# LouisBearing/BirdSoundClassif

Hardware: AMD Instinct MI355X
Metric: clips/sec (3 s @ 22.05 kHz) detect fwd (higher is better)
Workload: dtype f32; 1 GPU; BASELINE.json configs[1]: 1xMI355X inference, batch=64 synthetic 3 s clips (PCM16 @22.05 kHz resident in HBM) through the HIP STFT front end + detector forward + device post-processing, detections returned to the host; batch_per_gpu=64, distinct_clips=64, lanes=2

## Files before the change

### birdsoundclassif_amd/_lib.py

```python
import ctypes as C
import os
import subprocess

_HERE = os.path.dirname(os.path.abspath(__file__))
LIB_PATH = os.environ.get('NBM_LIB') or os.path.join(_HERE, 'libnbm_hip.so')
CSRC = os.path.join(_HERE, 'csrc')

_lib = None


class GemmDesc(C.Structure):
    _fields_ = [('x', C.c_void_p), ('w', C.c_void_p), ('y', C.c_void_p),
                ('scale', C.c_void_p), ('shift', C.c_void_p), ('residual', C.c_void_p),
                ('x_gs', C.c_int64), ('w_gs', C.c_int64), ('y_gs', C.c_int64), ('res_gs', C.c_int64),
                ('groups', C.c_int),
                ('B', C.c_int), ('H', C.c_int), ('W', C.c_int), ('Cin', C.c_int),
                ('N', C.c_int),
                ('kh', C.c_int), ('kw', C.c_int), ('stride', C.c_int), ('pad', C.c_int),
                ('Ho', C.c_int), ('Wo', C.c_int),
                ('x_ld', C.c_int), ('w_ld', C.c_int), ('y_ld', C.c_int), ('res_ld', C.c_int),
                ('alpha', C.c_float), ('act', C.c_int), ('shift_per_row', C.c_int),
                ('up', C.c_void_p), ('up_H', C.c_int), ('up_W', C.c_int),
                ('rows', C.c_void_p), ('rows_blocks', C.c_void_p),
                ('rows_mode', C.c_int), ('rows_count', C.c_int), ('rows_TH', C.c_int), ('rows_TW', C.c_int),
# ... 83 lines not shown
    'nbm_silu': [_P, _P, _L, _P],
    'nbm_layernorm': [_P, _L, _I, _P, _P, _F, _P, _P],
    'nbm_mha_small': [_P, _P, _P, _I, _I, _I, _P, _I, _I, _I, _I, _I, _L, _L, _P, _F, _P],
    'nbm_mha_segments': [_P, _P, _P, _I, _I, _I, _P, _I, _I, _I, _I, _I, _I, _P, _P, _I, _F, _P],
    'nbm_pair_softmax': [_P, _L, _I, _I, _P, _I, _P],
    'nbm_rpn_decode': [_P, _P, _P, _I, _I, _I, _I, _I, _I, _P, _P, _P, _P],
    'nbm_nan_images': [_P, _I, _L, _P, _P],
    'nbm_rpn_select': [_P, _P, _P, _I, _I, _I, _I, _I, _P, _P, _P, _P, _P],
    'nbm_nms_batched': [_P, _P, _P, _I, _I, _F, _I, _P, _P, _P, _P, _P, _P, _P],
    'nbm_rpn_select_big_workspace': [_I, _I, C.POINTER(C.c_int64)],
    'nbm_rpn_select_big': [_P, _P, _P, _I, _I, _I, _I, _I, _P, _L, _P, _P, _P, _P, _P],
    'nbm_nms_big_workspace': [_I, _I, C.POINTER(C.c_int64)],
    'nbm_nms_big': [_P, _P, _P, _I, _I, _F, _I, _P, _L, _P, _P, _P, _P, _P],
    'nbm_roi_pool': [C.POINTER(RoiDesc), _P],
    'nbm_roi_pool_hw': [C.POINTER(RoiHwDesc), _P],
    'nbm_rcnn_post': [_P, _P, _I, _I, _P, _P, _I, _I, _I, _F, _F, _I, _P, _P, _P],
    'nbm_merge_collect': [_P, _P, _I, _I, _I, _I, _I, _L, _P, _P, _P, _P, _P, _P],
    'nbm_merge_nms_workspace': [_I, C.POINTER(C.c_int64)],
    'nbm_merge_nms': [_P, _P, _I, _F, _P, _L, _P, _P, _P],
    'nbm_merge_gather': [_P, _P, _P, _P, _P, _I, _P, _P, _P],
    'nbm_conv_dgrad': [C.POINTER(BwdDesc), _P],
    'nbm_conv_wgrad': [C.POINTER(BwdDesc), _P],
    'nbm_gemm_plan': [_I, _P, C.POINTER(GemmPlan)],
    'nbm_relu_bwd': [_P, _P, _P, _L, _P],
    'nbm_silu_bwd': [_P, _P, _P, _L, _P],
    'nbm_axpby': [_P, _P, _P, _F, _F, _L, _L, _P],
    'nbm_colsum': [_P, _L, _I, _I, _P, _P],
    'nbm_leaky_relu_bwd': [_P, _P, _P, _F, _L, _P],
    'nbm_layernorm_bwd': [_P, _P, _P, _L, _I, _F, _P, _P, _P, _P],
    'nbm_mha_small_bwd': [_P, _P, _P, _P, _I, _I, _I, _I, _P, _P, _P, _I, _I, _I, _P, _I, _I, _I, _I, _L, _L, _P, _F, _P],
    'nbm_zero_roi_windows': [_P, _I, _I, _I, _P, _P, _I, _I, _I, _P],
    'nbm_zero_pattern': [_P, _I, _I, _I, _I, _I, _P],
    'nbm_zero_tiles': [_P, _I, _I, _I, _I, _P, _I, _P, _P],
    'nbm_tiles_gather': [_P, _I, _I, _I, _I, _P, _I, _P, _P, _P],
    'nbm_tiles_scatter_add': [_P, _I, _I, _I, _I, _P, _I, _P, _P, _P],
    'nbm_proposal_iou': [_P, _P, _P, _I, _I, _I, _P, _P, _P],
    'nbm_anchor_targets': [_P, _I, _P, _P, _I, _I, _F, _F, _P, _P, _P, _P],
    'nbm_maxpool3x3s2_bwd': [_P, _P, _P, _I, _I, _I, _I, _I, _I, _P, _P, _P],
    'nbm_upsample_bilinear_bwd': [_P, _I, _I, _I, _I, _P, _I, _I, _I, _P],
    'nbm_tiles_upsample_bilinear_bwd_add': [_P, _I, _I, _I, _I, _P, _I, _P, _P, _I, _I, _P],
    'nbm_png_unfilter_gray8': [_P, _L, _I, _I, _I, _P, _L, _P, _P],
    'nbm_image_half_std_u8': [_P, _L, _I, _L, _P, _P],
    'nbm_randn_fill': [_U64, _L, _P, _P],
    'nbm_augment_batch': [_P, _P, _P, _I, _I, _I, _P, _P, _P, _P, _P, _P, _P],
    'nbm_u8_to_unit': [_P, _L, _P, _P],
    'nbm_wino_input': [_P, _I, _I, _I, _I, _P, _I, _P],
# ... 48 lines not shown
def load():
    global _lib
    if _lib is not None:
        return _lib
    import torch
    if not os.path.isfile(LIB_PATH):
        raise RuntimeError(f'{LIB_PATH} is missing: build it with `python -c "import __graft_entry__ as g; g.build()"` '
                           '(the NBM hot path has no CPU / eager fallback)')
    lib = C.CDLL(LIB_PATH)
    lib.nbm_version.restype = C.c_char_p
    lib.nbm_version.argtypes = []
    for name, argtypes in SIGNATURES.items():
        fn = getattr(lib, name)
        fn.argtypes = argtypes
        fn.restype = C.c_int
    _lib = lib
    return lib


class NbmHipError(RuntimeError):
    pass


_CODES = {-1: 'NBM_EINVAL (bad argument / shape)', -2: 'NBM_EALIGN (pointer or pitch not 16-byte aligned)',
          -3: 'NBM_EUNSUPPORTED'}


def check(rc, name):
    if rc != 0:
        raise NbmHipError(f'{name} failed: {_CODES.get(rc, f"hipError_t {rc}")}')
```

### birdsoundclassif_amd/csrc/igemm.hip

```cpp
#include <stdlib.h>
#include "nbm_common.h"
#include "igemm_device.h"
#include <type_traits>

namespace {

constexpr int BK = 32;
constexpr int PITCH = 36;

enum { A_FAST = 0, A_GENERIC = 1 };

using nbm_igemm::IgemmParams;

template <int BM, int BN, int WM, int WN, int AMODE, int EPI, int STAGES = 2, bool ROWS = false>
__global__ __launch_bounds__(256, BM > 128 ? 1 : STAGES == 1 ? 3 : 2) void igemm_kernel(const IgemmParams p) {
  constexpr int MT = WM / 32, NT = WN / 32;
  constexpr int WAVES_N = BN / WN;
  constexpr int AR = BM / 32, BR = BN / 32;
  static_assert((BM / WM) * (BN / WN) == 4, "4 waves per workgroup");
  static_assert(EPI == EPI_STD, "EPI is reserved: the instantiation names carry it");

  __shared__ __attribute__((aligned(16))) float lds[STAGES * (BM + BN) * PITCH];
  if constexpr (STAGES == 2) nbm_stagger_priority();
  float* As = lds;
// ... 351 lines not shown
      }
    }
    if (p.bits_out) {
      static_assert(NT >= 2 && NT % 2 == 0, "two lanes per tile row");
      constexpr int WPL = NT / 2;
      __builtin_amdgcn_fence(__ATOMIC_ACQ_REL, "wavefront");
      const int r = lane >> 1, j0 = (lane & 1) * WPL;
      const int m = m0 + r;
      if (m < p.M) {
        unsigned* dst = p.bits_out + (long long)m * p.n_words + (n_off >> 5) + j0;
        const unsigned* src = Bw[wave] + r * NT + j0;
        if constexpr (WPL == 4) *reinterpret_cast<uint4*>(dst) = *reinterpret_cast<const uint4*>(src);
        else if constexpr (WPL == 2) *reinterpret_cast<uint2*>(dst) = *reinterpret_cast<const uint2*>(src);
        else {
#pragma unroll
          for (int q = 0; q < WPL; ++q) dst[q] = src[q];
        }
      }
      __builtin_amdgcn_fence(__ATOMIC_ACQ_REL, "wavefront");
    }
  }
}

}

using namespace nbm_igemm;

extern "C" int nbm_gemm_conv(const nbm_gemm_desc* d, void* stream) {
  if (!d) return NBM_EINVAL;
  const GemmPlan pl = plan_fwd(*d, read_gemm_switches(0));
  if (pl.rc) return pl.rc;
  if (pl.halves) {
    nbm_gemm_desc a = *d, b = *d;
    const int n0 = d->N - 64;
    a.N = n0;
    b.N = 64;
    b.w = d->w + (long long)n0 * d->w_ld;
    b.y = d->y + n0;
    if (d->scale) b.scale = d->scale + n0;
    if (d->shift) b.shift = d->shift + n0;
    if (d->residual) b.residual = d->residual + n0;
    if (d->mask) b.mask = d->mask + n0;
    const int rc = nbm_gemm_conv(&a, stream);
    return rc ? rc : nbm_gemm_conv(&b, stream);
  }
  const dim3 grid(pl.grid[0], pl.grid[1], pl.grid[2]), block(pl.block);
// ... 30 lines not shown
  }
  if (d->rows) {
    p.rows = d->rows; p.rows_blocks = d->rows_blocks; p.rows_mode = d->rows_mode; p.rows_TH = d->rows_TH; p.rows_TW = d->rows_TW;
    p.fd_rows_thw = nbm_fastdiv_make((unsigned)(d->rows_TH * d->rows_TW)); p.fd_rows_tw = nbm_fastdiv_make((unsigned)d->rows_TW);
    p.M = d->rows_count;
  }
  switch (pl.kernel) {
    case K_FWD_ROWS: hipLaunchKernelGGL((igemm_kernel<128, 128, 64, 64, A_FAST, EPI_STD, 1, true>), grid, block, 0, st, p); break;
    case K_FWD_SPLIT_R0: case K_FWD_SPLIT_R2: case K_FWD_SPLIT_R4: return split_launch(p, pl, st);
    case K_FWD_H16: return h16_launch(p, pl, st);
    case K_FWD_128_S1: hipLaunchKernelGGL((igemm_kernel<128, 128, 64, 64, A_FAST, EPI_STD, 1>), grid, block, 0, st, p); break;
    case K_FWD_128_FAST: hipLaunchKernelGGL((igemm_kernel<128, 128, 64, 64, A_FAST, EPI_STD>), grid, block, 0, st, p); break;
    case K_FWD_128_GENERIC: hipLaunchKernelGGL((igemm_kernel<128, 128, 64, 64, A_GENERIC, EPI_STD>), grid, block, 0, st, p); break;
    case K_FWD_64_S1: hipLaunchKernelGGL((igemm_kernel<128, 64, 64, 32, A_FAST, EPI_STD, 1>), grid, block, 0, st, p); break;
    case K_FWD_64_FAST: hipLaunchKernelGGL((igemm_kernel<128, 64, 64, 32, A_FAST, EPI_STD>), grid, block, 0, st, p); break;
    case K_FWD_64_GENERIC: hipLaunchKernelGGL((igemm_kernel<128, 64, 64, 32, A_GENERIC, EPI_STD>), grid, block, 0, st, p); break;
    case K_FWD_32_FAST: hipLaunchKernelGGL((igemm_kernel<128, 32, 32, 32, A_FAST, EPI_STD>), grid, block, 0, st, p); break;
    case K_FWD_32_GENERIC: hipLaunchKernelGGL((igemm_kernel<128, 32, 32, 32, A_GENERIC, EPI_STD>), grid, block, 0, st, p); break;
    default: return NBM_EINVAL;
  }
  return nbm_launch_status();
}

extern "C" int nbm_gemm_plan(int kind, const void* desc, nbm_gemm_plan_t* out) {
  if (!desc || !out || kind < 0 || kind > 2) return NBM_EINVAL;
  const GemmSwitches sw = read_gemm_switches(kind);
  *out = kind == 0 ? plan_fwd(*(const nbm_gemm_desc*)desc, sw)
         : kind == 1 ? plan_dgrad(*(const nbm_bwd_desc*)desc, sw) : plan_wgrad(*(const nbm_bwd_desc*)desc, sw);
  return out->rc;
}
```

### birdsoundclassif_amd/csrc/igemm_plan.h

```cpp
#pragma once
#include <stdint.h>
#include <stdlib.h>
#include "nbm_hip.h"

namespace nbm_igemm {

struct GemmSwitches { bool stream1x1, split_bf16, h16, nn_h16, split_tn; };
constexpr GemmSwitches kDefaultSwitches = {true, false, true, true, true};
inline bool switch_on(const char* v, bool dflt) { return dflt ? !(v && v[0] == '0') : (v && v[0] == '1'); }
inline GemmSwitches read_gemm_switches(int kind) {
  GemmSwitches s = kDefaultSwitches;
  if (kind == 0) {
    s.stream1x1 = switch_on(getenv("NBM_STREAM1X1"), true);
    s.split_bf16 = switch_on(getenv("NBM_SPLIT_BF16"), false);
    s.h16 = switch_on(getenv("NBM_H16"), true);
  } else if (kind == 1) {
    s.nn_h16 = switch_on(getenv("NBM_NN_H16"), true);
  } else {
    s.split_bf16 = switch_on(getenv("NBM_SPLIT_BF16"), false);
    s.split_tn = switch_on(getenv("NBM_SPLIT_TN"), true);
  }
  return s;
}

#define NBM_GEMM_KERNELS(X)                                                                                                          \
  X(K_FWD_ROWS, "igemm_kernel<128,128,64,64,0,0,1,true>")                                        \
  X(K_STREAM_64_256, "stream1x1_kernel<2,8,4,8>")                                          \
  X(K_STREAM_64_64, "stream1x1_kernel<2,2,2,8>")                                                \
  X(K_STREAM_256_64, "stream1x1_kernel<8,2,2,8>")                                                                     \
  X(K_STREAM_128_SLICED, "stream1x1_kernel<4,4,4,8>")                   \
  X(K_STREAM_256_SLICED, "stream1x1_kernel<8,2,2,8>")                     \
  X(K_FWD_SPLIT_R0, "igemm_split_kernel<0>")                                                        \
  X(K_FWD_SPLIT_R2, "igemm_split_kernel<2>")                                                                                         \
  X(K_FWD_SPLIT_R4, "igemm_split_kernel<4>")                                                                                         \
  X(K_FWD_H16, "igemm_h16_kernel")                                                                 \
  X(K_FWD_128_S1, "igemm_kernel<128,128,64,64,0,0,1,false>")                                              \
  X(K_FWD_128_FAST, "igemm_kernel<128,128,64,64,0,0,2,false>")                                                       \
  X(K_FWD_128_GENERIC, "igemm_kernel<128,128,64,64,1,0,2,false>")                                                                    \
  X(K_FWD_64_S1, "igemm_kernel<128,64,64,32,0,0,1,false>")                                                                           \
  X(K_FWD_64_FAST, "igemm_kernel<128,64,64,32,0,0,2,false>")                                                                         \
  X(K_FWD_64_GENERIC, "igemm_kernel<128,64,64,32,1,0,2,false>")                                                                      \
  X(K_FWD_32_FAST, "igemm_kernel<128,32,32,32,0,0,2,false>")                                                                         \
  X(K_FWD_32_GENERIC, "igemm_kernel<128,32,32,32,1,0,2,false>")                                                                      \
  X(K_NN_128_S1, "igemm_nn_kernel<128,1,false>")                                                                                     \
  X(K_NN_128_H16, "igemm_nn_kernel<128,2,true>")                                                                                     \
  X(K_NN_128, "igemm_nn_kernel<128,2,false>")                                                                                        \
  X(K_NN_64_S1, "igemm_nn_kernel<64,1,false>")                                                                                       \
  X(K_NN_64_H16, "igemm_nn_kernel<64,2,true>")                                                                                       \
  X(K_NN_64, "igemm_nn_kernel<64,2,false>")                                                                                          \
  X(K_TN_GENERIC, "igemm_tn_kernel<64,2,128>")                                                                                       \
  X(K_TN_128_SAME_M64, "igemm_tn_kernel<128,0,64>")                                                                                  \
  X(K_TN_128_STRIDED_M64, "igemm_tn_kernel<128,1,64>")                                                                               \
  X(K_TN_64_SAME_M64, "igemm_tn_kernel<64,0,64>")                                                                                    \
  X(K_TN_64_STRIDED_M64, "igemm_tn_kernel<64,1,64>")                                                                                 \
  X(K_TN_128_SAME, "igemm_tn_kernel<128,0,128>")                                                                                     \
  X(K_TN_128_STRIDED, "igemm_tn_kernel<128,1,128>")                                                                                  \
  X(K_TN_64_SAME, "igemm_tn_kernel<64,0,128>")                                                                                       \
  X(K_TN_64_STRIDED, "igemm_tn_kernel<64,1,128>")                                                                                    \
  X(K_SPLIT_TN_R0, "igemm_split_tn_kernel<0>")                              \
  X(K_SPLIT_TN_R2, "igemm_split_tn_kernel<2>")                                                                                       \
  X(K_SPLIT_TN_R4, "igemm_split_tn_kernel<4>")

enum GemmKernel {
#define X(id, name) id,
  NBM_GEMM_KERNELS(X)
#undef X
  K_COUNT
};
inline const char* gemm_kernel_name(int k) {
  static const char* const names[] = {
#define X(id, name) name,
      NBM_GEMM_KERNELS(X)
#undef X
  };
  return k >= 0 && k < K_COUNT ? names[k] : "";
}

constexpr int PLAN_BK = 32;
constexpr int SHORTK_STEPS = 8, DEEPK_STEPS = SHORTK_STEPS + 1;
constexpr int SHORTK_STEPS_64 = 20;
constexpr int SHORTK_STEPS_PHASED = 16;
constexpr int DEEPK_MAX_TAPS = 63;
constexpr int STREAM_MIN_ROWS = 8192;
constexpr int SPLIT_TN_MIN_ROWS = 192;
// ... 82 lines not shown
  }
  if (d.N > 64) {
    pl.n_tiles = (d.N + 127) / 128;
    const bool deep = fast_vec && nk >= DEEPK_STEPS && taps < DEEPK_MAX_TAPS;
    if (sw.split_bf16 && deep) {
      pl.m_tiles = (M + 255) / 256;
      const int rem = (2 * nk) % 6;
      plan_kernel(pl, rem == 0 ? K_FWD_SPLIT_R0 : rem == 2 ? K_FWD_SPLIT_R2 : K_FWD_SPLIT_R4, pl.m_tiles * pl.n_tiles, 1, d.groups);
    }
    else if (sw.h16 && deep) plan_kernel(pl, K_FWD_H16, pl.m_tiles * pl.n_tiles, 1, d.groups);
    else if (fast_vec && nk <= SHORTK_STEPS) plan_kernel(pl, K_FWD_128_S1, pl.m_tiles * pl.n_tiles, 1, d.groups);
    else plan_kernel(pl, pl.fast ? K_FWD_128_FAST : K_FWD_128_GENERIC, pl.m_tiles * pl.n_tiles, 1, d.groups);
  } else if (d.N > 32) {
    pl.n_tiles = 1;
    if (fast_vec && nk <= SHORTK_STEPS_64) plan_kernel(pl, K_FWD_64_S1, pl.m_tiles, 1, d.groups);
    else plan_kernel(pl, pl.fast ? K_FWD_64_FAST : K_FWD_64_GENERIC, pl.m_tiles, 1, d.groups);
  } else {
    pl.n_tiles = 1;
    plan_kernel(pl, pl.fast ? K_FWD_32_FAST : K_FWD_32_GENERIC, pl.m_tiles, 1, d.groups);
  }
  return pl;
}

inline int check_bwd_common(const nbm_bwd_desc& d) {
  if (!d.g || !d.out) return NBM_EINVAL;
  if (d.B <= 0 || d.H <= 0 || d.W <= 0 || d.Cin <= 0 || d.N <= 0 || d.kh <= 0 || d.kw <= 0 || d.stride <= 0 || d.groups <= 0 ||
      d.kh * d.kw > 64)
    return NBM_EINVAL;
  if ((d.H + 2 * d.pad - d.kh) / d.stride + 1 != d.Ho || (d.W + 2 * d.pad - d.kw) / d.stride + 1 != d.Wo) return NBM_EINVAL;
  return NBM_OK;
}

inline GemmPlan plan_dgrad(const nbm_bwd_desc& d, GemmSwitches sw) {
  if (int rc = check_bwd_common(d)) return plan_error(rc);
  if (!d.w) return plan_error(NBM_EINVAL);
  if ((d.g_ld & 3) || d.g_ld < ((d.N + 31) / 32) * 32 || (d.Cin & 3) || (d.w_ld & 3) || (d.g_gs & 3) || (d.w_gs & 3) || !aligned16(d.g) ||
      !aligned16(d.w) || (d.a_scale && !aligned16(d.a_scale)))
    return plan_error(NBM_EALIGN);
  if (d.out_ld < d.Cin || (d.residual && d.res_ld < d.Cin) || (d.mask && d.mask_ld < d.Cin)) return plan_error(NBM_EINVAL);
  if (d.residual2 && (d.stride != 1 || d.groups != 1 || d.res2_ld < d.Cin)) return plan_error(NBM_EINVAL);
  if (d.a_scale && (d.N & 31)) return plan_error(NBM_EINVAL);
  if (d.mask_bits && ((d.Cin & 31) || d.groups != 1)) return plan_error(NBM_EUNSUPPORTED);
  {
    const long long row = (long long)d.Wo * d.g_ld * 4;
    const long long span = (d.W == 1 && d.kh == 1) ? 130ll * d.g_ld * 4
                                                    : (d.kh + 130) * row + (long long)d.Ho * row;
// ... 92 lines not shown
```

### birdsoundclassif_amd/nets/backbone.py

```python
import torch
from torch import nn

from .. import ops
from . import _prep, functional as Fn
from .position_encoding import build_position_encoding

bcbk_channels = {'resnet': {'2': 64, '3': 256, '4': 512, '5': 1024, '6': 2048}}
_RESNET_LAYERS = {'resnet50': [3, 4, 6, 3], 'resnet101': [3, 4, 23, 3], 'resnet152': [3, 8, 36, 3]}
_RESNEXT = {'resnext50_32x4d': ([3, 4, 6, 3], 32, 4), 'resnext101_32x8d': ([3, 4, 23, 3], 32, 8),
            'resnext101_64x4d': ([3, 4, 23, 3], 64, 4)}


class FrozenBatchNorm2d(nn.Module):

    def __init__(self, n):
        super().__init__()
        self.register_buffer('weight', torch.ones(n))
        self.register_buffer('bias', torch.zeros(n))
        self.register_buffer('running_mean', torch.zeros(n))
        self.register_buffer('running_var', torch.ones(n))

    def _load_from_state_dict(self, state_dict, prefix, local_metadata, strict, missing_keys, unexpected_keys,
                              error_msgs):
        state_dict.pop(prefix + 'num_batches_tracked', None)
# ... 12 lines not shown
        self.bn1 = norm_layer(planes)
        self.conv2 = nn.Conv2d(planes, planes, 3, stride=stride, padding=1, bias=False)
        self.bn2 = norm_layer(planes)
        self.conv3 = nn.Conv2d(planes, planes * 4, 1, bias=False)
        self.bn3 = norm_layer(planes * 4)
        self.downsample = downsample
        self.stride = stride
        self.mask_input, self.mask_gy = False, True

    def forward(self, x):
        if torch.is_grad_enabled() and x.dim() == 4 and self.conv1.weight.shape[0] % 32 == 0:
            ds = self.downsample
            sd, bd = ds[1].affine() if ds is not None else (None, None)
            return Fn.Bottleneck.apply(x, self.conv1.weight, self.conv2.weight, self.conv3.weight,
                                       ds[0].weight if ds is not None else None, *self.bn1.affine(), *self.bn2.affine(),
                                       *self.bn3.affine(), sd, bd, self.stride, self.mask_input, self.mask_gy)
        s, b = self.bn1.affine()
        o = Fn.conv(x, self.conv1.weight, scale=s, shift=b, act=ops.ACT_RELU)
        s, b = self.bn2.affine()
        if self.stride == 1 and Fn._winograd_ok(o, self.conv2.weight, 3, 3, 1, 1):
            o = ops.conv3x3_winograd(o, _prep.wino23(self.conv2.weight), b, scale=s, relu=True)
        else:
            o = Fn.conv(o, self.conv2.weight, scale=s, shift=b, kh=3, kw=3, stride=self.stride, pad=1, act=ops.ACT_RELU)
        if self.downsample is not None:
            s, b = self.downsample[1].affine()
            idt = Fn.conv(x, self.downsample[0].weight, scale=s, shift=b, stride=self.stride)
        else:
            idt = x
        s, b = self.bn3.affine()
        return Fn.conv(o, self.conv3.weight, scale=s, shift=b, residual=idt, act=ops.ACT_RELU)


class _GroupedBottleneck(nn.Module):

    def __init__(self, inplanes, planes, stride, downsample, norm_layer, groups, base_width):
        super().__init__()
        width = int(planes * base_width / 64) * groups
        self.conv1 = nn.Conv2d(inplanes, width, 1, bias=False)
        self.bn1 = norm_layer(width)
        self.conv2 = nn.Conv2d(width, width, 3, stride=stride, padding=1, groups=groups, bias=False)
        self.bn2 = norm_layer(width)
        self.conv3 = nn.Conv2d(width, planes * 4, 1, bias=False)
        self.bn3 = norm_layer(planes * 4)
        self.downsample = downsample
        self.stride, self.groups = stride, groups
        self.mask_input, self.mask_gy = False, True
# ... 120 lines not shown
```

### birdsoundclassif_amd/nets/functional.py

```python
import os
import weakref

import torch
from torch.autograd import Function
from torch.autograd.function import once_differentiable

from .. import ops, ondemand
from . import _prep

ACT_NONE, ACT_RELU, ACT_LEAKY = ops.ACT_NONE, ops.ACT_RELU, ops.ACT_LEAKY


def _pad32_rows(g2d, n):
    n32 = (n + 31) // 32 * 32
    if n32 == n:
        return g2d
    out = torch.zeros((g2d.shape[0], n32), device=g2d.device, dtype=torch.float32)
    out[:, :n] = g2d
    return out


GRAD_SINK = {}


# ... 568 lines not shown
        y = ops.stem7x7(x, *_prep.stem_fold(w1, w_init, b_init), scale, shift)
        ctx.save_for_backward(x, w_init, b_init, w1, scale, y)
        return y

    @staticmethod
    @once_differentiable
    def backward(ctx, gy):
        x, w_init, b_init, w1, scale, y = ctx.saved_tensors
        g = gy.contiguous() if _premasked(y, gy) else ops.relu_bwd(gy.contiguous(), y)
        U, V = ops.stem7x7_wgrad(x, g)
        U, V = U * scale.view(64, 1, 1), V * scale.view(64, 1, 1)
        wi, bi = w_init.detach().view(3), b_init.detach().view(3)
        gw1 = wi.view(1, 3, 1, 1) * U[:, None] + bi.view(1, 3, 1, 1) * V[:, None]
        w1d = w1.detach()
        gwi = (w1d * U[:, None]).sum(dim=(0, 2, 3)).view_as(w_init)
        gbi = (w1d * V[:, None]).sum(dim=(0, 2, 3))
        return None, gwi, gbi, gw1, None, None


class MaxPool(Function):

    @staticmethod
    def forward(ctx, x, relu_input=False):
        y, idx = ops.maxpool3x3s2(x, with_index=True)
        ctx.hw = x.shape[1:3]
        ctx.x_ptr, ctx.take_x = x.data_ptr(), stash_accept(x, ctx.needs_input_grad[0])
        ctx.premask = bool(relu_input and ctx.take_x)
        ctx.save_for_backward(idx, x if ctx.premask else None)
        return y

    @staticmethod
    @once_differentiable
    def backward(ctx, gy):
        idx, x = ctx.saved_tensors
        other = _STASH.pop(ctx.x_ptr, None) if ctx.take_x else None
        premask = ctx.premask and other is not None
        gx = ops.maxpool3x3s2_bwd(idx, gy.contiguous(), *ctx.hw, residual=other, mask=x if premask else None)
        ondemand.zero_recycle(other)
        if premask:
            _PREMASKED[ctx.x_ptr] = (gx.data_ptr(), gx._version)
        return gx, None


class SpaceToBatch2(Function):

    @staticmethod
# ... 409 lines not shown
```

### birdsoundclassif_amd/ops.py

```python
import collections
import ctypes as C
import os
import math

import torch

from . import _lib
from ._lib import GconvBwdDesc, GconvDesc, GemmDesc, RoiDesc, RoiHwDesc, check

ACT_NONE, ACT_RELU, ACT_SILU, ACT_LEAKY = 0, 1, 2, 3

PROFILE = None
FLOPS = None
FLOPS_DEFERRED = []


def flops_total():
    tot = FLOPS[0] + sum(float(c.item()) * f for c, f in FLOPS_DEFERRED)
    FLOPS_DEFERRED.clear()
    return tot


_PROFILE_LABEL = None
PROFILE_ONLY = None
# ... 14 lines not shown

def _stream():
    return C.c_void_p(torch.cuda.current_stream().cuda_stream)


def _ptr(t):
    return C.c_void_p(t.data_ptr()) if t is not None else C.c_void_p(0)


def _chk(t, dtype=torch.float32, name='tensor'):
    if not (isinstance(t, torch.Tensor) and t.is_cuda):
        raise RuntimeError(f'{name}: the NBM HIP path needs CUDA (ROCm) tensors; no CPU fallback exists')
    if t.dtype != dtype:
        raise TypeError(f'{name}: expected {dtype}, got {t.dtype}')
    if not t.is_contiguous():
        raise ValueError(f'{name}: must be contiguous')
    return t


def lib():
    return _lib.load()


def gemm_conv(x, w, y, *, B, H, W, Cin, N, kh=1, kw=1, stride=1, pad=0, Ho=None, Wo=None,
              x_ld=None, w_ld=None, y_ld=None, scale=None, shift=None, residual=None, res_ld=None,
              groups=1, x_gs=0, w_gs=0, y_gs=0, res_gs=0, alpha=1.0, act=ACT_NONE, shift_per_row=False, up=None,
              rows=None, rows_mode=0, rows_count=0, rows_blocks=None, rows_thw=(0, 0), mask=None, mask_ld=None, bits_out=None):
    Ho = (H + 2 * pad - kh) // stride + 1 if Ho is None else Ho
    Wo = (W + 2 * pad - kw) // stride + 1 if Wo is None else Wo
    d = GemmDesc()
    d.x, d.w, d.y = x.data_ptr(), w.data_ptr(), y.data_ptr()
    d.scale = scale.data_ptr() if scale is not None else None
    d.shift = shift.data_ptr() if shift is not None else None
    d.residual = residual.data_ptr() if residual is not None else None
    d.x_gs, d.w_gs, d.y_gs, d.res_gs = x_gs, w_gs, y_gs, res_gs
    d.groups = groups
    d.B, d.H, d.W, d.Cin, d.N = B, H, W, Cin, N
    d.kh, d.kw, d.stride, d.pad, d.Ho, d.Wo = kh, kw, stride, pad, Ho, Wo
    d.x_ld = Cin if x_ld is None else x_ld
    d.w_ld = kh * kw * Cin if w_ld is None else w_ld
    d.y_ld = N if y_ld is None else y_ld
    d.res_ld = (N if res_ld is None else res_ld) if residual is not None else 0
    d.alpha, d.act, d.shift_per_row = float(alpha), int(act), int(bool(shift_per_row))
    if up is not None:
        d.up, d.up_H, d.up_W = _chk(up, name='up').data_ptr(), up.shape[1], up.shape[2]
    if mask is not None:
        d.mask, d.mask_ld = mask.data_ptr(), int(N if mask_ld is None else mask_ld)
    if bits_out is not None:
        assert bits_out.dtype == torch.int32 and bits_out.is_contiguous() and bits_out.numel() * 32 >= B * Ho * Wo * N and N % 32 == 0
        d.bits_out = bits_out.data_ptr()
    if rows is not None:
        d.rows, d.rows_mode, d.rows_count = rows.data_ptr(), int(rows_mode), int(rows_count)
        d.rows_blocks = rows_blocks.data_ptr() if rows_blocks is not None else None
        d.rows_TH, d.rows_TW = rows_thw
    if FLOPS is not None:
        if rows is None:
            FLOPS[0] += 2.0 * B * Ho * Wo * N * kh * kw * Cin * groups
        elif rows_blocks is None:
            FLOPS[0] += 2.0 * rows_count * N * Cin
        else:
            FLOPS_DEFERRED.append((rows_blocks.clone(), 2.0 * 128 * (16 if rows_mode == 2 else 1) * N * Cin))
    if _prof_all() or (PROFILE is not None and PROFILE_ONLY == 'deepk' and is_deepk(Cin, N, kh, kw, rows)):
        ev0, ev1 = torch.cuda.Event(enable_timing=True), torch.cuda.Event(enable_timing=True)
        ev0.record()
        check(lib().nbm_gemm_conv(C.byref(d), _stream()), 'nbm_gemm_conv')
        ev1.record()
        if rows is None:
            PROFILE.append(((Cin, N, kh, H, W, B, groups, stride, _PROFILE_LABEL), ev0, ev1))
        elif rows_blocks is None:
            PROFILE.append(((Cin, N, kh, rows_count, 1, 1, groups, stride, ('rows', H, W)), ev0, ev1))
        else:
            PROFILE.append(((Cin, N, kh, 0, 1, 1, groups, stride, ('rows-rois', H, W)), ev0, ev1))
        return y
    check(lib().nbm_gemm_conv(C.byref(d), _stream()), 'nbm_gemm_conv')
    return y


def conv2d(x, w, kh=1, kw=1, stride=1, pad=0, scale=None, shift=None, residual=None, act=ACT_NONE,
           alpha=1.0, out=None, w_ld=None, up=None, bits_out=None):
    _chk(x, name='x'), _chk(w, name='w')
    B, H, W, Cin = x.shape
    N = w.shape[0]
    Ho = (H + 2 * pad - kh) // stride + 1
    Wo = (W + 2 * pad - kw) // stride + 1
    y = out if out is not None else torch.empty((B, Ho, Wo, N), device=x.device, dtype=torch.float32)
    if residual is not None:
        _chk(residual, name='residual')
        assert residual.shape == y.shape
    gemm_conv(x, w, y, B=B, H=H, W=W, Cin=Cin, N=N, kh=kh, kw=kw, stride=stride, pad=pad, Ho=Ho, Wo=Wo,
              w_ld=w.shape[1] if w_ld is None else w_ld, scale=scale, shift=shift, residual=residual,
              alpha=alpha, act=act, up=up, bits_out=bits_out)
    return y


def gconv3x3(x, w_prepared, groups, stride=1, scale=None, shift=None, relu=False, out=None, kh=3, kw=3, pad=1):
    _chk(x, name='x'), _chk(w_prepared, name='w_prepared')
    if x.dim() != 4 or w_prepared.dim() != 5 or tuple(w_prepared.shape[1::2]) != (9, 64) or w_prepared.shape[4] != 4 or groups <= 0 \
            or (16 * w_prepared.shape[0]) % groups:
# ... 825 lines not shown
PROFILE_BWD = None


def _bwd_desc(g, *, B, H, W, Cin, N, kh, kw, stride, pad, g_ld, groups=1, alpha=1.0):
    d = BwdDesc()
    d.g = g.data_ptr()
    d.groups = groups
    d.B, d.H, d.W, d.Cin, d.N = B, H, W, Cin, N
    d.kh, d.kw, d.stride, d.pad = kh, kw, stride, pad
    d.Ho = (H + 2 * pad - kh) // stride + 1
    d.Wo = (W + 2 * pad - kw) // stride + 1
    d.g_ld = g_ld
    d.alpha = float(alpha)
    return d


GemmPlan = collections.namedtuple('GemmPlan', 'rc kernel grid block m_tiles n_tiles vec_epi fast slices phased ph_tiles splits k_chunk '
                                              'plain b_generic narrow_m halves')


def gemm_plan(kind, desc):
    p = _lib.GemmPlan()
    lib().nbm_gemm_plan(int(kind), C.byref(desc), C.byref(p))
    return GemmPlan(p.rc, (p.name or b'').decode(), tuple(p.grid), p.block, p.m_tiles, p.n_tiles, p.vec_epi, p.fast, p.slices, p.phased,
                    tuple(p.ph_tiles), p.splits, p.k_chunk, p.plain, p.b_generic, p.narrow_m, p.halves)


def split_nn():
    return os.environ.get('NBM_SPLIT_BF16') == '1' and os.environ.get('NBM_SPLIT_NN', '1') != '0'


def conv_dgrad(g, w, out, *, B, H, W, Cin, N, kh=1, kw=1, stride=1, pad=0, g_ld=None, w_ld=None, out_ld=None,
               a_scale=None, residual=None, mask=None, alpha=1.0, groups=1, g_gs=0, w_gs=0, out_gs=0, res_gs=0, residual2=None,
               mask_bits=None):
    if (kh == 1 and kw == 1 and stride == 1 and pad == 0 and residual2 is None and N > 256 and N % 32 == 0 and Cin > 64 and Cin % 4 == 0 and
            (groups == 1 or (mask is None and a_scale is None)) and split_nn()):
        wl = kh * kw * Cin if w_ld is None else w_ld
        wv = w.as_strided((groups, N, Cin), (w_gs, wl, 1))
        wt = (wv * a_scale[None, :N, None] if a_scale is not None else wv).transpose(1, 2).contiguous()
        with _timed(('dgrad', B, H, W, Cin, N, kh, stride, groups)):
            gemm_conv(g, wt, out, B=B, H=H, W=W, Cin=N, N=Cin, x_ld=N if g_ld is None else g_ld, w_ld=N,
                      y_ld=Cin if out_ld is None else out_ld, residual=residual, res_ld=Cin if residual is not None else None, alpha=alpha,
                      mask=mask, mask_ld=Cin if mask is not None else None, groups=groups, x_gs=g_gs, w_gs=Cin * N, y_gs=out_gs, res_gs=res_gs)
        return out
    d = _bwd_desc(g, B=B, H=H, W=W, Cin=Cin, N=N, kh=kh, kw=kw, stride=stride, pad=pad,
                  g_ld=N if g_ld is None else g_ld, groups=groups, alpha=alpha)
# ... 405 lines not shown
```

### include/nbm_hip.h

```cpp
#ifndef NBM_HIP_H
#define NBM_HIP_H

#include <stdint.h>

#ifdef __cplusplus
extern "C" {
#endif

#define NBM_OK 0
#define NBM_EINVAL (-1)
#define NBM_EALIGN (-2)
#define NBM_EUNSUPPORTED (-3)

#define NBM_ACT_NONE 0
#define NBM_ACT_RELU 1
#define NBM_ACT_SILU 2
#define NBM_ACT_LEAKY 3

const char* nbm_version(void);

int nbm_graph_census(void* graph, long long counts[6]);

typedef struct nbm_gemm_desc {
  const float* x;
// ... 271 lines not shown
  int res2_ld;
  const unsigned* mask_bits;
} nbm_bwd_desc;

int nbm_conv_dgrad(const nbm_bwd_desc* d, void* stream);
int nbm_conv_wgrad(const nbm_bwd_desc* d, void* stream);

typedef struct nbm_gemm_plan_t {
  const char* name;
  int rc;
  int kernel;
  int grid[3], block;
  int m_tiles, n_tiles;
  int vec_epi;
  int fast;
  int slices;
  int phased;
  int ph_tiles[4];
  int splits, k_chunk;
  int plain, b_generic, narrow_m;
  int halves;
} nbm_gemm_plan_t;
int nbm_gemm_plan(int kind, const void* desc, nbm_gemm_plan_t* out);

int nbm_relu_bwd(const float* gy, const float* y, float* out, int64_t n, void* stream);
int nbm_silu_bwd(const float* gy, const float* x, float* out, int64_t n, void* stream);
int nbm_axpby(const float* a, const float* b, float* out, float alpha, float beta, int64_t n, int64_t b_period, void* stream);
int nbm_weighted_sum(const float* x0, const float* x1, const float* x2, const float* weights, float* out, int64_t n,
                     void* stream);
int nbm_weighted_sum_bwd(const float* x0, const float* x1, const float* x2, const float* weights, const float* g, float* gx0,
                         float* gx1, float* gx2, float* gw, int64_t n, void* stream);
int nbm_zero_roi_windows(float* g, int H, int W, int C, const float* rois , const int* level ,
                         int B, int n_roi, int lvl, void* stream);
int nbm_zero_pattern(float* g, int B, int H, int W, int C, int stride, void* stream);
int nbm_zero_tiles(float* g, int B, int H, int W, int C, const int* tiles, int n_entries, const int* n_blocks, void* stream);
int nbm_tiles_gather(const float* map, int B, int H, int W, int C, const int* tiles, int n_entries, const int* n_blocks, float* compact,
                     void* stream);
int nbm_tiles_scatter_add(float* map, int B, int H, int W, int C, const int* tiles, int n_entries, const int* n_blocks,
                          const float* compact, void* stream);
int nbm_colsum(const float* g, int64_t M, int N, int ld, float* out, void* stream);
int nbm_maxpool3x3s2_bwd(const uint8_t* idx, const float* gy, float* gx, int B, int H, int W, int C, int Ho, int Wo,
                         const float* residual ,
                         const float* mask ,
                         void* stream);
int nbm_leaky_relu_bwd(const float* gy, const float* y, float* out, float slope, int64_t n, void* stream);
int nbm_layernorm_bwd(const float* x, const float* w, const float* g, int64_t rows, int E, float eps, float* gx, float* gw,
// ... 55 lines not shown
```

Before: 1089 clips/s.

## Fuse bottleneck conv3 and downsample 1x1 convs into one paired stream kernel

Adds a stream1x1 pair kernel that computes both the main-branch conv3 (1x1, 64->256) and the downsample shortcut 1x1 conv in one launch. It applies both BN affines, adds them and applies ReLU in the epilogue, so the shortcut output is never written to and re-read from global memory. The ResNet bottleneck forward uses it for stride-1 downsample blocks under no-grad, and falls back to two convs when the planner rejects the shape. Separately, maxpool skips computing argmax indices when no gradient is needed. The risk is that the fused kernel holds more registers and LDS, which could lower occupancy.

After: 1088 clips/s. No clear change (-0.0%).

```diff
diff --git a/birdsoundclassif_amd/_lib.py b/birdsoundclassif_amd/_lib.py
--- a/birdsoundclassif_amd/_lib.py
+++ b/birdsoundclassif_amd/_lib.py
@@ -129,6 +129,8 @@
     'nbm_conv_dgrad': [C.POINTER(BwdDesc), _P],
     'nbm_conv_wgrad': [C.POINTER(BwdDesc), _P],
     'nbm_gemm_plan': [_I, _P, C.POINTER(GemmPlan)],
+    'nbm_gemm_conv_pair': [C.POINTER(GemmDesc), C.POINTER(GemmDesc), _P],
+    'nbm_gemm_pair_plan': [C.POINTER(GemmDesc), C.POINTER(GemmDesc), C.POINTER(GemmPlan)],
     'nbm_relu_bwd': [_P, _P, _P, _L, _P],
     'nbm_silu_bwd': [_P, _P, _P, _L, _P],
     'nbm_axpby': [_P, _P, _P, _F, _F, _L, _L, _P],
@@ -223,6 +225,7 @@
     pass
 
 
+EUNSUPPORTED = -3
 _CODES = {-1: 'NBM_EINVAL (bad argument / shape)', -2: 'NBM_EALIGN (pointer or pitch not 16-byte aligned)',
           -3: 'NBM_EUNSUPPORTED'}
 
diff --git a/birdsoundclassif_amd/csrc/igemm.hip b/birdsoundclassif_amd/csrc/igemm.hip
--- a/birdsoundclassif_amd/csrc/igemm.hip
+++ b/birdsoundclassif_amd/csrc/igemm.hip
@@ -397,6 +397,139 @@
   }
 }
 
+struct StreamPairParams {
+  const float* x; const float* w; const float* scale; const float* shift;
+  const float* xd; const float* wd; const float* scale_d; const float* shift_d;
+  float* y;
+  int M, x_ld, w_ld, xd_ld, wd_ld, y_ld, m_tiles; float alpha, alpha_d; int act;
+  unsigned* bits_out; int n_words;
+};
+template <int NT, int NTG, int WAVES>
+__global__ __launch_bounds__(WAVES * 64, 1) void stream1x1_pair_kernel(const StreamPairParams p) {
+  constexpr int K32 = 2, K = K32 * 32, N = NT * 32, WP = K + 4;
+  static_assert(NT % NTG == 0, "groups");
+  __shared__ __attribute__((aligned(16))) float Ws[2][N * WP];
+  __shared__ __attribute__((aligned(16))) float Stg[WAVES][32 * SPITCH];
+  __shared__ __attribute__((aligned(16))) unsigned Bw[WAVES][32 * NT];
+  __shared__ __attribute__((aligned(16))) float Aff[4][N];
+  const int tid = threadIdx.x, lane = tid & 63, wave = tid >> 6, li = lane & 31, lh = lane >> 5;
+  const int n_off = blockIdx.y * N;
+  for (int i = tid; i < N * (K / 4); i += WAVES * 64) {
+    const int n = i / (K / 4), c = i - n * (K / 4);
+    *reinterpret_cast<f32x4*>(Ws[0] + n * WP + c * 4) = *reinterpret_cast<const f32x4*>(p.w + (long long)(n_off + n) * p.w_ld + c * 4);
+    *reinterpret_cast<f32x4*>(Ws[1] + n * WP + c * 4) = *reinterpret_cast<const f32x4*>(p.wd + (long long)(n_off + n) * p.wd_ld + c * 4);
+  }
+  for (int i = tid; i < N; i += WAVES * 64) {
+    Aff[0][i] = p.scale ? p.scale[n_off + i] : 1.f;
+    Aff[1][i] = p.shift ? p.shift[n_off + i] : 0.f;
+    Aff[2][i] = p.scale_d ? p.scale_d[n_off + i] : 1.f;
+    Aff[3][i] = p.shift_d ? p.shift_d[n_off + i] : 0.f;
+  }
+  __syncthreads();
+  float* stg = Stg[wave];
+  const int er = lane >> 3, ec = (lane & 7) * 4;
+  f32x4 a[K32][4], an[K32][4], ad[K32][4], adn[K32][4];
+  auto load_rows = [&](int tile, f32x4 (*dst)[4], f32x4 (*dst_d)[4]) {
+    int m = tile * 32 + li;
+    m = m < p.M ? m : p.M - 1;
+    const float* xp = p.x + (long long)m * p.x_ld + 16 * lh;
+    const float* xq = p.xd + (long long)m * p.xd_ld + 16 * lh;
+#pragma unroll
+    for (int kc = 0; kc < K32; ++kc)
+#pragma unroll
+      for (int q = 0; q < 4; ++q) dst[kc][q] = *reinterpret_cast<const f32x4*>(xp + kc * 32 + 4 * q);
+#pragma unroll
+    for (int kc = 0; kc < K32; ++kc)
+#pragma unroll
+      for (int q = 0; q < 4; ++q) dst_d[kc][q] = *reinterpret_cast<const f32x4*>(xq + kc * 32 + 4 * q);
+  };
+  auto mfma_block = [&](const float* wb, const f32x4 (*src)[4], f32x16& acc) {
+#pragma unroll
+    for (int kc = 0; kc < K32; ++kc) {
+      f32x4 b[4];
+#pragma unroll
+      for (int q = 0; q < 4; ++q) b[q] = *reinterpret_cast<const f32x4*>(wb + kc * 32 + 4 * q);
+#pragma unroll
+      for (int q = 0; q < 4; ++q)
+#pragma unroll
+        for (int e = 0; e < 4; ++e) acc = __builtin_amdgcn_mfma_f32_32x32x2f32(src[kc][q][e], b[q][e], acc, 0, 0, 0);
+    }
+  };
+  const int step = gridDim.x * WAVES;
+  int tile = blockIdx.x * WAVES + wave;
+  if (tile < p.m_tiles) load_rows(tile, an, adn);
+  for (; tile < p.m_tiles; tile += step) {
+    const bool more = tile + step < p.m_tiles;
+#pragma unroll
+    for (int kc = 0; kc < K32; ++kc)
+#pragma unroll
+      for (int q = 0; q < 4; ++q) { a[kc][q] = an[kc][q]; ad[kc][q] = adn[kc][q]; }
+    load_rows(more ? tile + step : tile, an, adn);
+    const int m0 = tile * 32;
+#pragma unroll
+    for (int g = 0; g < NT / NTG; ++g) {
+      f32x16 acc[NTG], acc_d[NTG];
+#pragma unroll
+      for (int j = 0; j < NTG; ++j)
+#pragma unroll
+        for (int e = 0; e < 16; ++e) acc[j][e] = acc_d[j][e] = 0.f;
+#pragma unroll
+      for (int j = 0; j < NTG; ++j) mfma_block(Ws[1] + ((g * NTG + j) * 32 + li) * WP + 16 * lh, ad, acc_d[j]);
+#pragma unroll
+      for (int j = 0; j < NTG; ++j) mfma_block(Ws[0] + ((g * NTG + j) * 32 + li) * WP + 16 * lh, a, acc[j]);
+#pragma unroll
+      for (int j = 0; j < NTG; ++j) {
+        const int jj = g * NTG + j;
+        const int n = n_off + jj * 32 + ec;
+        f32x4 sc = *reinterpret_cast<const f32x4*>(Aff[2] + jj * 32 + ec), sh = *reinterpret_cast<const f32x4*>(Aff[3] + jj * 32 + ec);
+        __builtin_amdgcn_fence(__ATOMIC_ACQ_REL, "wavefront");
+#pragma unroll
+        for (int e = 0; e < 16; ++e) stg[((e & 3) + 8 * (e >> 2) + 4 * lh) * SPITCH + li] = acc_d[j][e];
+        __builtin_amdgcn_fence(__ATOMIC_ACQ_REL, "wavefront");
+        f32x4 idt[4];
+#pragma unroll
+        for (int pass = 0; pass < 4; ++pass)
+          idt[pass] = epi_affine4(*reinterpret_cast<const f32x4*>(stg + (pass * 8 + er) * SPITCH + ec), p.alpha_d, sc, sh, 0.f);
+        __builtin_amdgcn_fence(__ATOMIC_ACQ_REL, "wavefront");
+#pragma unroll
+        for (int e = 0; e < 16; ++e) stg[((e & 3) + 8 * (e >> 2) + 4 * lh) * SPITCH + li] = acc[j][e];
+        __builtin_amdgcn_fence(__ATOMIC_ACQ_REL, "wavefront");
+        sc = *reinterpret_cast<const f32x4*>(Aff[0] + jj * 32 + ec), sh = *reinterpret_cast<const f32x4*>(Aff[1] + jj * 32 + ec);
+#pragma unroll
+        for (int pass = 0; pass < 4; ++pass) {
+          const int r = pass * 8 + er, m = m0 + r;
+          if (m >= p.M) continue;
+          f32x4 v = epi_affine4(*reinterpret_cast<const f32x4*>(stg + r * SPITCH + ec), p.alpha, sc, sh, 0.f);
+          {
+#pragma clang fp contract(off)
+            v[0] += idt[pass][0]; v[1] += idt[pass][1]; v[2] += idt[pass][2]; v[3] += idt[pass][3];
+          }
+          v = epi_act4(v, p.act);
+          if (p.bits_out) {
+            const unsigned wb = epi_relu_bits(v, 8 * er);
+            if (ec == 0) Bw[wave][r * NT + jj] = wb;
+          }
+          *reinterpret_cast<f32x4*>(p.y + (long long)m * p.y_ld + n) = v;
+        }
+      }
+    }
+    if (p.bits_out) {
+      static_assert(NT == 4 || NT == 8, "two lanes per tile row, 8- or 16-byte pieces");
+      constexpr int WPL = NT / 2;
+      __builtin_amdgcn_fence(__ATOMIC_ACQ_REL, "wavefront");
+      const int r = lane >> 1, j0 = (lane & 1) * WPL;
+      const int m = m0 + r;
+      if (m < p.M) {
+        unsigned* dst = p.bits_out + (long long)m * p.n_words + (n_off >> 5) + j0;
+        const unsigned* src = Bw[wave] + r * NT + j0;
+        if constexpr (WPL == 4) *reinterpret_cast<uint4*>(dst) = *reinterpret_cast<const uint4*>(src);
+        else *reinterpret_cast<uint2*>(dst) = *reinterpret_cast<const uint2*>(src);
+      }
+      __builtin_amdgcn_fence(__ATOMIC_ACQ_REL, "wavefront");
+    }
+  }
+}
+
 }
 
 using namespace nbm_igemm;
@@ -473,6 +606,23 @@
   return nbm_launch_status();
 }
 
+extern "C" int nbm_gemm_conv_pair(const nbm_gemm_desc* main, const nbm_gemm_desc* shortcut, void* stream) {
+  if (!main || !shortcut) return NBM_EINVAL;
+  const GemmPlan pl = plan_pair(*main, *shortcut, read_gemm_switches(3));
+  if (pl.rc) return pl.rc;
+  const StreamPairParams sp{main->x, main->w, main->scale, main->shift, shortcut->x, shortcut->w, shortcut->scale, shortcut->shift,
+                            main->y, main->B * main->Ho * main->Wo, main->x_ld, main->w_ld, shortcut->x_ld, shortcut->w_ld, main->y_ld,
+                            pl.m_tiles, main->alpha, shortcut->alpha, main->act, main->bits_out, main->N >> 5};
+  hipLaunchKernelGGL((stream1x1_pair_kernel<4, 2, 8>), dim3(pl.grid[0], pl.grid[1], pl.grid[2]), dim3(pl.block), 0, (hipStream_t)stream, sp);
+  return nbm_launch_status();
+}
+
+extern "C" int nbm_gemm_pair_plan(const nbm_gemm_desc* main, const nbm_gemm_desc* shortcut, nbm_gemm_plan_t* out) {
+  if (!main || !shortcut || !out) return NBM_EINVAL;
+  *out = plan_pair(*main, *shortcut, read_gemm_switches(3));
+  return out->rc;
+}
+
 extern "C" int nbm_gemm_plan(int kind, const void* desc, nbm_gemm_plan_t* out) {
   if (!desc || !out || kind < 0 || kind > 2) return NBM_EINVAL;
   const GemmSwitches sw = read_gemm_switches(kind);
diff --git a/birdsoundclassif_amd/csrc/igemm_plan.h b/birdsoundclassif_amd/csrc/igemm_plan.h
--- a/birdsoundclassif_amd/csrc/igemm_plan.h
+++ b/birdsoundclassif_amd/csrc/igemm_plan.h
@@ -5,8 +5,8 @@
 
 namespace nbm_igemm {
 
-struct GemmSwitches { bool stream1x1, split_bf16, h16, nn_h16, split_tn; };
-constexpr GemmSwitches kDefaultSwitches = {true, false, true, true, true};
+struct GemmSwitches { bool stream1x1, split_bf16, h16, nn_h16, split_tn, stream_pair; };
+constexpr GemmSwitches kDefaultSwitches = {true, false, true, true, true, true};
 inline bool switch_on(const char* v, bool dflt) { return dflt ? !(v && v[0] == '0') : (v && v[0] == '1'); }
 inline GemmSwitches read_gemm_switches(int kind) {
   GemmSwitches s = kDefaultSwitches;
@@ -16,6 +16,9 @@
     s.h16 = switch_on(getenv("NBM_H16"), true);
   } else if (kind == 1) {
     s.nn_h16 = switch_on(getenv("NBM_NN_H16"), true);
+  } else if (kind == 3) {
+    s.stream1x1 = switch_on(getenv("NBM_STREAM1X1"), true);
+    s.stream_pair = switch_on(getenv("NBM_STREAM_PAIR"), true);
   } else {
     s.split_bf16 = switch_on(getenv("NBM_SPLIT_BF16"), false);
     s.split_tn = switch_on(getenv("NBM_SPLIT_TN"), true);
@@ -59,7 +62,8 @@
   X(K_TN_64_STRIDED, "igemm_tn_kernel<64,1,128>")                                                                                    \
   X(K_SPLIT_TN_R0, "igemm_split_tn_kernel<0>")                              \
   X(K_SPLIT_TN_R2, "igemm_split_tn_kernel<2>")                                                                                       \
-  X(K_SPLIT_TN_R4, "igemm_split_tn_kernel<4>")
+  X(K_SPLIT_TN_R4, "igemm_split_tn_kernel<4>")                                                                                       \
+  X(K_STREAM_PAIR_64_256, "stream1x1_pair_kernel<4,2,8>")
 
 enum GemmKernel {
 #define X(id, name) id,
@@ -188,6 +192,32 @@
   return pl;
 }
 
+inline GemmPlan plan_pair(const nbm_gemm_desc& main, const nbm_gemm_desc& shortcut, GemmSwitches sw) {
+  nbm_gemm_desc sc = shortcut;
+  sc.y = main.y;
+  sc.y_ld = main.y_ld;
+  const nbm_gemm_desc* both[2] = {&main, &sc};
+  for (const nbm_gemm_desc* d : both) {
+    const GemmPlan one = plan_fwd(*d, sw);
+    if (one.rc) return one;
+    if (one.halves || !one.fast || !one.vec_epi || d->kh != 1 || d->kw != 1 || d->stride != 1 || d->pad != 0 || d->groups != 1 || d->up ||
+        d->mask || d->rows || d->shift_per_row || d->residual || d->Cin != 64 || d->N != 256)
+      return plan_error(NBM_EUNSUPPORTED);
+  }
+  const int M = main.B * main.Ho * main.Wo;
+  if (!sw.stream1x1 || !sw.stream_pair || sc.B != main.B || sc.Ho != main.Ho || sc.Wo != main.Wo || sc.act != NBM_ACT_NONE || sc.bits_out ||
+      M < STREAM_MIN_ROWS)
+    return plan_error(NBM_EUNSUPPORTED);
+  GemmPlan pl{};
+  pl.vec_epi = pl.fast = 1;
+  const int waves = 8, slices = 2;
+  pl.m_tiles = (M + 31) / 32;
+  pl.slices = slices;
+  const int wgs = (pl.m_tiles + waves - 1) / waves, gx = 256 / slices;
+  plan_kernel(pl, K_STREAM_PAIR_64_256, wgs < gx ? wgs : gx, slices, 1, waves * 64);
+  return pl;
+}
+
 inline int check_bwd_common(const nbm_bwd_desc& d) {
   if (!d.g || !d.out) return NBM_EINVAL;
   if (d.B <= 0 || d.H <= 0 || d.W <= 0 || d.Cin <= 0 || d.N <= 0 || d.kh <= 0 || d.kw <= 0 || d.stride <= 0 || d.groups <= 0 ||
diff --git a/birdsoundclassif_amd/nets/backbone.py b/birdsoundclassif_amd/nets/backbone.py
--- a/birdsoundclassif_amd/nets/backbone.py
+++ b/birdsoundclassif_amd/nets/backbone.py
@@ -58,6 +58,11 @@
             o = ops.conv3x3_winograd(o, _prep.wino23(self.conv2.weight), b, scale=s, relu=True)
         else:
             o = Fn.conv(o, self.conv2.weight, scale=s, shift=b, kh=3, kw=3, stride=self.stride, pad=1, act=ops.ACT_RELU)
+        if self.downsample is not None and self.stride == 1 and not torch.is_grad_enabled():
+            s, b = self.bn3.affine()
+            sd, bd = self.downsample[1].affine()
+            return ops.conv2d_pair(o, _prep.krsc(self.conv3.weight), x, _prep.krsc(self.downsample[0].weight), scale=s, shift=b,
+                                   scale_d=sd, shift_d=bd, act=ops.ACT_RELU)
         if self.downsample is not None:
             s, b = self.downsample[1].affine()
             idt = Fn.conv(x, self.downsample[0].weight, scale=s, shift=b, stride=self.stride)
diff --git a/birdsoundclassif_amd/nets/functional.py b/birdsoundclassif_amd/nets/functional.py
--- a/birdsoundclassif_amd/nets/functional.py
+++ b/birdsoundclassif_amd/nets/functional.py
@@ -614,6 +614,8 @@
 
     @staticmethod
     def forward(ctx, x, relu_input=False):
+        if not ctx.needs_input_grad[0]:
+            return ops.maxpool3x3s2(x)
         y, idx = ops.maxpool3x3s2(x, with_index=True)
         ctx.hw = x.shape[1:3]
         ctx.x_ptr, ctx.take_x = x.data_ptr(), stash_accept(x, ctx.needs_input_grad[0])
diff --git a/birdsoundclassif_amd/ops.py b/birdsoundclassif_amd/ops.py
--- a/birdsoundclassif_amd/ops.py
+++ b/birdsoundclassif_amd/ops.py
@@ -60,14 +60,14 @@
     return _lib.load()
 
 
-def gemm_conv(x, w, y, *, B, H, W, Cin, N, kh=1, kw=1, stride=1, pad=0, Ho=None, Wo=None,
+def gemm_desc(x, w, y, *, B, H, W, Cin, N, kh=1, kw=1, stride=1, pad=0, Ho=None, Wo=None,
               x_ld=None, w_ld=None, y_ld=None, scale=None, shift=None, residual=None, res_ld=None,
               groups=1, x_gs=0, w_gs=0, y_gs=0, res_gs=0, alpha=1.0, act=ACT_NONE, shift_per_row=False, up=None,
               rows=None, rows_mode=0, rows_count=0, rows_blocks=None, rows_thw=(0, 0), mask=None, mask_ld=None, bits_out=None):
     Ho = (H + 2 * pad - kh) // stride + 1 if Ho is None else Ho
     Wo = (W + 2 * pad - kw) // stride + 1 if Wo is None else Wo
     d = GemmDesc()
-    d.x, d.w, d.y = x.data_ptr(), w.data_ptr(), y.data_ptr()
+    d.x, d.w, d.y = x.data_ptr(), w.data_ptr(), (y.data_ptr() if y is not None else None)
     d.scale = scale.data_ptr() if scale is not None else None
     d.shift = shift.data_ptr() if shift is not None else None
     d.residual = residual.data_ptr() if residual is not None else None
@@ -91,6 +91,14 @@
         d.rows, d.rows_mode, d.rows_count = rows.data_ptr(), int(rows_mode), int(rows_count)
         d.rows_blocks = rows_blocks.data_ptr() if rows_blocks is not None else None
         d.rows_TH, d.rows_TW = rows_thw
+    return d
+
+
+def gemm_conv(x, w, y, *, B, H, W, Cin, N, kh=1, kw=1, stride=1, pad=0, Ho=None, Wo=None, groups=1, rows=None, rows_mode=0,
+              rows_count=0, rows_blocks=None, **kw_desc):
+    d = gemm_desc(x, w, y, B=B, H=H, W=W, Cin=Cin, N=N, kh=kh, kw=kw, stride=stride, pad=pad, Ho=Ho, Wo=Wo, groups=groups, rows=rows,
+                  rows_mode=rows_mode, rows_count=rows_count, rows_blocks=rows_blocks, **kw_desc)
+    Ho, Wo = d.Ho, d.Wo
     if FLOPS is not None:
         if rows is None:
             FLOPS[0] += 2.0 * B * Ho * Wo * N * kh * kw * Cin * groups
@@ -112,6 +120,46 @@
         return y
     check(lib().nbm_gemm_conv(C.byref(d), _stream()), 'nbm_gemm_conv')
     return y
+
+
+def gemm_conv_pair(main, shortcut):
+    B, H, W, N = main.B, main.Ho, main.Wo, main.N
+    prof = _prof_all()
+    if prof:
+        ev0, ev1 = torch.cuda.Event(enable_timing=True), torch.cuda.Event(enable_timing=True)
+        ev0.record()
+    rc = lib().nbm_gemm_conv_pair(C.byref(main), C.byref(shortcut), _stream())
+    if rc == _lib.EUNSUPPORTED:
+        return False
+    check(rc, 'nbm_gemm_conv_pair')
+    if FLOPS is not None:
+        FLOPS[0] += 2.0 * B * H * W * N * (main.Cin + shortcut.Cin)
+    if prof:
+        ev1.record()
+        PROFILE.append(((main.Cin + shortcut.Cin, N, 1, H, W, B, 1, 1, 'pair'), ev0, ev1))
+    return True
+
+
+def gemm_pair_plan(main, shortcut):
+    p = _lib.GemmPlan()
+    lib().nbm_gemm_pair_plan(C.byref(main), C.byref(shortcut), C.byref(p))
+    return _plan_tuple(p)
+
+
+def conv2d_pair(x, w, xd, wd, scale=None, shift=None, scale_d=None, shift_d=None, act=ACT_NONE, alpha=1.0, out=None, bits_out=None):
+    _chk(x, name='x'), _chk(w, name='w'), _chk(xd, name='xd'), _chk(wd, name='wd')
+    B, H, W, Cin = x.shape
+    N = w.shape[0]
+    if xd.shape[:3] != x.shape[:3] or wd.shape[0] != N:
+        raise ValueError('conv2d_pair: the two branches must share the pixel grid and the output channels')
+    y = out if out is not None else torch.empty((B, H, W, N), device=x.device, dtype=torch.float32)
+    main = gemm_desc(x, w, y, B=B, H=H, W=W, Cin=Cin, N=N, w_ld=w.shape[1], scale=scale, shift=shift, alpha=alpha, act=act,
+                     bits_out=bits_out)
+    short = gemm_desc(xd, wd, None, B=B, H=H, W=W, Cin=xd.shape[3], N=N, w_ld=wd.shape[1], scale=scale_d, shift=shift_d)
+    if gemm_conv_pair(main, short):
+        return y
+    idt = conv2d(xd, wd, scale=scale_d, shift=shift_d)
+    return conv2d(x, w, scale=scale, shift=shift, residual=idt, act=act, alpha=alpha, out=y, bits_out=bits_out)
 
 
 def conv2d(x, w, kh=1, kw=1, stride=1, pad=0, scale=None, shift=None, residual=None, act=ACT_NONE,
@@ -983,6 +1031,10 @@
 def gemm_plan(kind, desc):
     p = _lib.GemmPlan()
     lib().nbm_gemm_plan(int(kind), C.byref(desc), C.byref(p))
+    return _plan_tuple(p)
+
+
+def _plan_tuple(p):
     return GemmPlan(p.rc, (p.name or b'').decode(), tuple(p.grid), p.block, p.m_tiles, p.n_tiles, p.vec_epi, p.fast, p.slices, p.phased,
                     tuple(p.ph_tiles), p.splits, p.k_chunk, p.plain, p.b_generic, p.narrow_m, p.halves)
 
diff --git a/include/nbm_hip.h b/include/nbm_hip.h
--- a/include/nbm_hip.h
+++ b/include/nbm_hip.h
@@ -317,6 +317,9 @@
   int halves;
 } nbm_gemm_plan_t;
 int nbm_gemm_plan(int kind, const void* desc, nbm_gemm_plan_t* out);
+
+int nbm_gemm_conv_pair(const nbm_gemm_desc* main, const nbm_gemm_desc* shortcut, void* stream);
+int nbm_gemm_pair_plan(const nbm_gemm_desc* main, const nbm_gemm_desc* shortcut, nbm_gemm_plan_t* out);
 
 int nbm_relu_bwd(const float* gy, const float* y, float* out, int64_t n, void* stream);
 int nbm_silu_bwd(const float* gy, const float* x, float* out, int64_t n, void* stream);
```
